# OpenDriveLab/Vista

Measured on AMD Instinct MI355X. Metric: denoise steps/sec, 25-frame 576x1024 latent, 50-step EDM @ 1/2/4/8 GPU, higher is better.
Workload: dtype bf16; 1 GPU; 1xMI355X single GPU: 25x576x1024 (latent 25x4x72x128), 50-step EulerEDM, VanillaCFG 2.5 (N=50 images per UNet call), bf16, random-init 1.65B VideoUNet, synthetic latents; frames=25, cfg_images_per_call=50, sampler=EulerEDM s_churn=0, 50-step schedule, parallelism=single GPU

## Files before the change

include/vista_hip.h:

```cpp
#ifndef VISTA_HIP_H
#define VISTA_HIP_H
#include <stdint.h>
#ifdef __cplusplus
extern "C" {
#endif

enum { VK_AMODE_DENSE = 0, VK_AMODE_CONV3X3 = 1, VK_AMODE_TEMPORAL3 = 2, VK_AMODE_CONV3D = 3 };
enum { VK_EPI_LINEAR = 0, VK_EPI_GEGLU = 1, VK_EPI_TRANS = 2 };

typedef struct VkGemmDesc {
    const void* A;
    const void* Wt;
    void* out;
    const float* bias;
    const float* rowvec;
    const void* res1;
    const void* res2;
    int32_t M, N, K;
    int32_t lda, ldc, ld_res1, ld_res2, ldv, rows_per_vec;
    float alpha, beta;
    int32_t amode, epi, out_f32;
    int32_t H, Wd, Cin, Hout, Wout, stride, ups;
    int32_t T, S;
    int32_t tile_cfg;
// ... 46 lines not shown
int vk_ff_fused_bf16(const VkGemmDesc* geglu, const VkGemmDesc* out_proj, void* stream);
int vk_ff_fused_rowstat_parts(void);

int vk_groupnorm_silu_fp8(const void* x1, const void* x2, void* y8, float* scale_out, const float* gamma, const float* beta, float* stats_ws,
                          int32_t n_img, int32_t S, int32_t C1, int32_t C2, int32_t frames_per_group, float eps, int32_t silu, void* stream);

int vk_layernorm_quant_fp8(const void* x, void* q, float* scale, const float* gamma, const float* beta, int32_t rows, int32_t C, float eps,
                           void* stream);

int vk_quantize_rows_fp8(const void* x, void* q, float* scale, int32_t M, int32_t K, int64_t ldx, int64_t ldq, void* stream);

int vk_attn_spatial_bf16(const void* q, const void* k, const void* vt, void* o, int32_t n_img, int32_t heads,
                         int32_t S, int32_t ldq, int32_t ldk, int32_t ldo, float scale, void* stream);

int vk_attn_spatial_qkv_bf16(const void* q, const void* k, const void* v, void* o, int32_t n_img, int32_t heads,
                             int32_t S, int32_t ldq, int32_t ldk, int32_t ldv, int32_t ldo, float scale, void* stream);

int vk_attn_spatial_qkv_log2_bf16(const void* q, const void* k, const void* v, void* o, int32_t n_img, int32_t heads,
                                  int32_t S, int32_t ldq, int32_t ldk, int32_t ldv, int32_t ldo, void* stream);

int vk_attn_small_bf16(const void* qkv, void* o, int32_t n_img, int32_t heads, int32_t S, int32_t D, int32_t ld, int32_t k_off,
                       int32_t v_off, int32_t ldo, float scale, void* stream);

int vk_clip_preprocess_patches(const float* img, void* out, int32_t n_img, int32_t H, int32_t W, int32_t out_hw, int32_t patch, int32_t ldo,
                               float sigma_y, float sigma_x, int32_t ks_y, int32_t ks_x, const float* mean3, const float* std3, void* stream);

int vk_attn_spatial_fp8qk(const void* q8, const void* k8, const void* q_scales, const void* k_scales, const void* v, void* o, void* o8,
                          void* o_scales, int32_t n_img, int32_t heads, int32_t S, int32_t ldq8, int32_t ldk8, int32_t ldqs, int32_t ldks,
                          int32_t ldv, int32_t ldo, int32_t ldo8, int32_t ldos, float scale, void* stream);

int vk_attn_temporal_bf16(const void* qkv, void* o, int32_t B, int32_t T, int32_t S, int32_t heads, int32_t ld,
                          int32_t k_off, int32_t v_off, int32_t ldo, float scale, void* stream);

int vk_softmax_rows_f32_bf16(const float* x, void* y, int64_t rows, int32_t cols, int64_t ldx, int64_t ldy, void* stream);

int vk_groupnorm_silu_bf16(const void* x, void* y, const float* gamma, const float* beta, float* stats_ws,
                           int32_t n_img, int32_t S, int32_t C, int32_t frames_per_group, float eps, int32_t silu,
                           void* stream);

int vk_groupnorm_stats_bf16(const void* x, float* sums, float* partial_ws, int32_t n_img, int32_t S, int32_t C,
                            int32_t frames_per_group, void* stream);
int vk_groupnorm_apply_bf16(const void* x, void* y, const float* gamma, const float* beta, const float* sums, int32_t n_img,
                            int32_t S, int32_t C, int32_t frames_per_group, float count, float eps, int32_t silu, void* stream);
int vk_groupnorm_finalize_partials(float* partial, float* sums, int32_t n_img, int32_t nchunks, int32_t frames_per_group, void* stream);
int vk_groupnorm_fold_max(void);
int vk_groupnorm_apply_partials_bf16(const void* x, void* y, const float* gamma, const float* beta, const float* partial, int32_t n_img,
                                     int32_t S, int32_t C, int32_t nchunks, int32_t frames_per_group, float count, float eps, int32_t silu,
                                     void* stream);

int vk_layernorm_bf16(const void* x, void* y, void* sum_out, const float* gamma, const float* beta,
                      const float* addvec, int32_t rows, int32_t C, int32_t rows_per_vec, int32_t ldv, float eps,
                      void* stream);

int vk_rowstats_bf16(const void* x, float* stats, int32_t rows, int32_t C, int64_t ldx, void* stream);

int vk_groupnorm_silu_cat_bf16(const void* x1, const void* x2, void* y, const float* gamma, const float* beta, float* stats_ws,
                               int32_t n_img, int32_t S, int32_t C1, int32_t C2, int32_t frames_per_group, float eps, int32_t silu,
                               void* stream);

int vk_concat_channels_bf16(const void* a, const void* b, void* out, int64_t rows, int32_t C1, int32_t C2, void* stream);

int vk_nchw_to_tokens_bf16(const float* x, void* out, int32_t n_img, int32_t C, int32_t HW, int32_t Cpad, void* stream);
int vk_tokens_to_nchw_f32(const float* x, float* out, int32_t n_img, int32_t C, int32_t HW, int32_t ldx, void* stream);

int vk_timestep_embedding_bf16(const float* t, void* out, int32_t n, int32_t dim, float max_period, void* stream);
int vk_timestep_embedding_f32(const float* t, float* out, int32_t n, int32_t dim, float max_period, void* stream);
// ... 59 lines not shown
```

vista_amd/_lib.py:

```python
import ctypes as C
import os

_HERE = os.path.dirname(os.path.abspath(__file__))
ACT_DTYPE = os.environ.get("VISTA_ACT_DTYPE", "bf16").lower()
if ACT_DTYPE not in ("bf16", "fp16"):
    raise ValueError(f"VISTA_ACT_DTYPE must be 'bf16' or 'fp16', not {ACT_DTYPE!r}")
CURRENT = ACT_DTYPE
_LIB_FILES = {"bf16": "libvista_hip.so", "fp16": "libvista_hip_f16.so"}
LIB_PATH = os.environ.get("VISTA_HIP_LIB") or os.path.join(_HERE, "lib", _LIB_FILES[ACT_DTYPE])


def lib_path(dtype_name):
    return LIB_PATH if dtype_name == ACT_DTYPE else os.path.join(_HERE, "lib", _LIB_FILES[dtype_name])


_vp = C.c_void_p
_i32 = C.c_int32
_i64 = C.c_int64
_f32 = C.c_float


class VkFp8Args(C.Structure):
    _fields_ = [("a_scale", _vp), ("w_scale", _vp), ("k_real", _i32), ("a_mx", _vp), ("ld_mx", _i32), ("mx_out", _vp), ("ld_mx_out", _i32),
                ("a_scale_rows", _i32)]
# ... 23 lines not shown

class VkRowBox(C.Structure):
    _fields_ = [("src_row", _i64), ("dst_row", _i64), ("src_stride_b", _i64), ("src_stride_t", _i64), ("dst_stride_b", _i64), ("dst_stride_t", _i64),
                ("nb", _i32), ("nt", _i32), ("ns", _i32), ("reserved", _i32)]


class VkRowBoxes(C.Structure):
    _fields_ = [("n", _i32), ("reserved", _i32), ("box", VkRowBox * VK_RESHARD_MAX_BOXES)]


ABI_VERSION = 9

SIGNATURES = {
    "vk_gemm_bf16": [C.POINTER(VkGemmDesc), _vp],
    "vk_gemm_rowstat_parts": [C.POINTER(VkGemmDesc)],
    "vk_gemm_tile_choice": [C.POINTER(VkGemmDesc)],
    "vk_gemm_tail_split": [C.POINTER(VkGemmDesc)],
    "vk_gemm_gnstat_fit": [C.POINTER(VkGemmDesc)],
    "vk_gemm_fp8": [C.POINTER(VkGemmDesc), _vp, _vp, _i32, _vp],
    "vk_gemm_fp8_mx": [C.POINTER(VkGemmDesc), C.POINTER(VkFp8Args), _vp],
    "vk_gemm_fp8_rowstat_parts": [C.POINTER(VkGemmDesc)],
    "vk_ff_fused_bf16": [C.POINTER(VkGemmDesc), C.POINTER(VkGemmDesc), _vp],
    "vk_ff_fused_rowstat_parts": [],
    "vk_layernorm_quant_fp8": [_vp, _vp, _vp, _vp, _vp, _i32, _i32, _f32, _vp],
    "vk_groupnorm_silu_fp8": [_vp, _vp, _vp, _vp, _vp, _vp, _vp, _i32, _i32, _i32, _i32, _i32, _f32, _i32, _vp],
    "vk_quantize_rows_fp8": [_vp, _vp, _vp, _i32, _i32, _i64, _i64, _vp],
    "vk_attn_spatial_bf16": [_vp, _vp, _vp, _vp, _i32, _i32, _i32, _i32, _i32, _i32, _f32, _vp],
    "vk_attn_spatial_qkv_bf16": [_vp, _vp, _vp, _vp, _i32, _i32, _i32, _i32, _i32, _i32, _i32, _f32, _vp],
    "vk_attn_spatial_qkv_log2_bf16": [_vp, _vp, _vp, _vp, _i32, _i32, _i32, _i32, _i32, _i32, _i32, _vp],
    "vk_attn_spatial_fp8qk": [_vp, _vp, _vp, _vp, _vp, _vp, _vp, _vp, _i32, _i32, _i32, _i32, _i32, _i32, _i32, _i32, _i32, _i32, _i32, _f32, _vp],
    "vk_attn_small_bf16": [_vp, _vp, _i32, _i32, _i32, _i32, _i32, _i32, _i32, _i32, _f32, _vp],
    "vk_clip_preprocess_patches": [_vp, _vp, _i32, _i32, _i32, _i32, _i32, _i32, _f32, _f32, _i32, _i32, C.POINTER(_f32), C.POINTER(_f32), _vp],
    "vk_attn_temporal_bf16": [_vp, _vp, _i32, _i32, _i32, _i32, _i32, _i32, _i32, _i32, _f32, _vp],
    "vk_softmax_rows_f32_bf16": [_vp, _vp, _i64, _i32, _i64, _i64, _vp],
    "vk_groupnorm_silu_bf16": [_vp, _vp, _vp, _vp, _vp, _i32, _i32, _i32, _i32, _f32, _i32, _vp],
    "vk_groupnorm_stats_bf16": [_vp, _vp, _vp, _i32, _i32, _i32, _i32, _vp],
    "vk_groupnorm_apply_bf16": [_vp, _vp, _vp, _vp, _vp, _i32, _i32, _i32, _i32, _f32, _f32, _i32, _vp],
    "vk_groupnorm_finalize_partials": [_vp, _vp, _i32, _i32, _i32, _vp],
    "vk_groupnorm_fold_max": [],
    "vk_groupnorm_apply_partials_bf16": [_vp, _vp, _vp, _vp, _vp, _i32, _i32, _i32, _i32, _i32, _f32, _f32, _i32, _vp],
    "vk_layernorm_bf16": [_vp, _vp, _vp, _vp, _vp, _vp, _i32, _i32, _i32, _i32, _f32, _vp],
    "vk_rowstats_bf16": [_vp, _vp, _i32, _i32, _i64, _vp],
    "vk_groupnorm_silu_cat_bf16": [_vp, _vp, _vp, _vp, _vp, _vp, _i32, _i32, _i32, _i32, _i32, _f32, _i32, _vp],
    "vk_concat_channels_bf16": [_vp, _vp, _vp, _i64, _i32, _i32, _vp],
    "vk_nchw_to_tokens_bf16": [_vp, _vp, _i32, _i32, _i32, _i32, _vp],
    "vk_tokens_to_nchw_f32": [_vp, _vp, _i32, _i32, _i32, _i32, _vp],
    "vk_timestep_embedding_bf16": [_vp, _vp, _i32, _i32, _f32, _vp],
    "vk_timestep_embedding_f32": [_vp, _vp, _i32, _i32, _f32, _vp],
    "vk_emb_combine": [_vp, _vp, _vp, _vp, _vp, _vp, _i32, _i32, _vp],
    "vk_silu_f32_to_bf16": [_vp, _vp, _i64, _vp],
    "vk_cast_f32_to_bf16": [_vp, _vp, _i64, _vp],
    "vk_sampler_prepare": [_vp, _vp, _vp, _vp, _vp, _vp, _i32, _i32, _i32, _f32, _i32, _vp],
    "vk_sampler_update": [_vp, _vp, _vp, _i32, _i32, _i32, _f32, _f32, _f32, _f32, _vp],
    "vk_denoiser_combine": [_vp, _vp, _vp, _vp, _vp, _i32, _i32, _vp],
    "vk_cfg_combine": [_vp, _vp, _vp, _i32, _i32, _vp],
    "vk_euler_step": [_vp, _vp, _vp, _vp, _vp, _i32, _i32, _vp],
    "vk_mask_replace": [_vp, _vp, _vp, _vp, _i32, _i32, _vp],
    "vk_scale_rows": [_vp, _vp, _vp, _i32, _i32, _vp],
    "vk_gaussian_sample": [_vp, _vp, _vp, _i32, _i32, _i32, _f32, _vp],
    "vk_ensemble_variance_sum": [_vp, _vp, _vp, _i32, _i64, _vp],
    "vk_lanczos_resize_u8": [_vp, _vp, _vp, _vp, _vp, _i32, _vp, _vp, _i32, _vp, _i32, _i32, _i32, _i32, _i32, _i32, _i32, _i32, _i32, _vp],
    "vk_frames_to_u8": [_vp, _vp, _i32, _i32, _i32, _i32, _i32, _i32, _vp],
    "vk_ensemble_frame_stats": [_vp, _vp, _vp, _vp, _i32, _i32, _i32, _i32, _vp],
    "vk_heat_overlay_u8": [_vp, _vp, _vp, _i32, _i32, _i32, _i32, _f32, _f32, _vp],
    "vk_copy_row_boxes": [_vp, _vp, C.POINTER(VkRowBoxes), _i64, _i64, _i32, _vp],
    "vk_abi_version": [],
# ... 39 lines not shown
```

vista_amd/build.py:

```python
import os
import subprocess
import sys

ROOT = os.path.dirname(os.path.abspath(__file__))
REPO = os.path.dirname(ROOT)
CSRC = os.path.join(ROOT, "csrc")
LIBDIR = os.path.join(ROOT, "lib")
LIB = os.path.join(LIBDIR, "libvista_hip.so")
EXTRA_FLAGS = {"ff_fused.hip": ["-fno-slp-vectorize"], "attention.hip": ["-fno-slp-vectorize"]}
SOURCES = ["gemm.hip", "gemm_pipe.hip", "gemm_pipe2.hip", "gemm_stream.hip", "gemm_fp8.hip", "ff_fused.hip", "attention.hip", "norm.hip", "elementwise.hip", "image_io.hip", "reshard.hip", "reward.hip"]


def hipcc():
    for c in (os.environ.get("HIPCC"), "/opt/rocm/bin/hipcc", "hipcc"):
        if c and (os.path.isabs(c) and os.path.exists(c) or not os.path.isabs(c)):
            return c
    raise RuntimeError("hipcc not found")


VARIANTS = {"bf16": ("libvista_hip.so", "", []), "fp16": ("libvista_hip_f16.so", "_f16", ["-DVK_F16=1"])}
LIB_F16 = os.path.join(LIBDIR, VARIANTS["fp16"][0])


def needs_build(lib=LIB):
    if not os.path.exists(lib):
        return True
    t = os.path.getmtime(lib)
    deps = [os.path.join(CSRC, f) for f in os.listdir(CSRC)] + [os.path.join(REPO, "include", "vista_hip.h")]
    return any(os.path.getmtime(d) > t for d in deps)


def build(force=False, verbose=True, variants=("bf16", "fp16")):
    os.makedirs(LIBDIR, exist_ok=True)
    procs, links = [], []
    for v in variants:
        libname, suffix, defs = VARIANTS[v]
        lib = os.path.join(LIBDIR, libname)
        if not force and not needs_build(lib):
            continue
        objs = []
        for s in SOURCES:
            o = os.path.join(LIBDIR, s.replace(".hip", suffix + ".o"))
            cmd = [hipcc(), "--offload-arch=gfx950", "-O3", "-std=c++17", "-fPIC", "-I" + os.path.join(REPO, "include"),
# ... 28 lines not shown
```

vista_amd/modules/diffusionmodules/sampling.py:

```python
import os
from typing import Dict, Union

import torch

from ... import ops
from ...util import append_dims, default, instantiate_from_config
from .guiders import IdentityGuider


class FusedDenoiser:

    def __init__(self, denoiser, network):
        self.denoiser, self.network = denoiser, network

    def __call__(self, x, sigma, cond, cond_mask):
        return self.denoiser(self.network, x, sigma, cond, cond_mask)


class BaseDiffusionSampler:
    def __init__(self, discretization_config: Union[Dict, None], num_steps: Union[int, None] = None,
                 guider_config: Union[Dict, None] = None, verbose: bool = False, device: str = "cuda"):
        self.num_steps = num_steps
        self.discretization = instantiate_from_config(discretization_config)
        self.guider = instantiate_from_config(default(guider_config, {"target": "vista_amd.modules.diffusionmodules.guiders.IdentityGuider"}))
# ... 51 lines not shown
                and self._fused_layout_ok(denoiser, x, cond, uc):
            return self._sample_fused(denoiser, x, cond, uc, cond_frame, maskf, replace, sig)
        n = x.shape[0]
        xw = x.float()
        for i in range(num_sigmas - 1):
            if replace:
                xw = ops.mask_replace(xw, cond_frame.float(), maskf)
            gamma = min(self.s_churn / (num_sigmas - 1), 2 ** 0.5 - 1) if self.s_tmin <= sig[i] <= self.s_tmax else 0.0
            s_cur = torch.full((n,), sig[i], device=x.device)
            s_next = torch.full((n,), sig[i + 1], device=x.device)
            xw = self.sampler_step(s_cur, s_next, denoiser, xw, cond, maskf, uc, gamma)
        if replace:
            xw = ops.mask_replace(xw, cond_frame.float(), maskf)
        return xw.to(x.dtype)

    @staticmethod
    def _fused_layout_ok(fd, x, cond, uc):
        if x.dim() != 4 or x.shape[1] != 4 or getattr(fd.network.diffusion_model, "in_channels", None) != 8:
            return False
        for d in (cond, uc):
            if d is None or any(k not in d for k in ("concat", "crossattn", "vector")):
                return False
            c = d["concat"]
            if c.dim() != 4 or tuple(c.shape[1:]) != tuple(x.shape[1:]):
                return False
        return True

    def _sample_fused(self, fd, x, cond, uc, cond_frame, maskf, replace, sig):
        loop = FusedLoop(self, fd, x.float().clone(), cond, uc, cond_frame, maskf, replace, sig, shard=getattr(self, "shard", None),
                         graph=self.graph, cfg_streams=self.cfg_streams)
        for i in range(len(sig) - 1):
            loop.step(i)
        return loop.finish().to(x.dtype)


class FusedLoop:

    def __init__(self, sampler, fd, xw, cond, uc, cond_frame, maskf, replace, sig, shard=None, graph=None, cfg_streams=None):
        from .video_model import CIN_PAD
        self.cin_pad = CIN_PAD
        import os
        want = os.environ.get("VISTA_HIPGRAPH", "0") if graph is None else ("1" if graph else "0")
        self._graph_mode = want
        self._graph = None
        self.den, self.unet = fd.denoiser, fd.network.diffusion_model
        self.sig, self.replace, self.shard = sig, replace, shard
        n, _, self.H, self.W = xw.shape
        self.n, self.T = n, self.den.num_frames
        T, dev = self.T, xw.device
        scales = sampler.guider.frame_scales(T).float().repeat(n // T).to(dev)
        if shard is not None and n != T:
            raise NotImplementedError("frame sharding handles one window (b = 1) per call")
        loc = (lambda t: t) if shard is None else (lambda t: shard.take_local_frames(t).contiguous())
        self.xw, self.maskf, self.scales = loc(xw), loc(maskf), loc(scales)

        def both(k):
            a, b = uc[k], cond[k]
            if a.shape[0] != n:
                a, b = a.repeat_interleave(T, 0), b.repeat_interleave(T, 0)
            return a, b
        cu, cc = both("concat")
        self.cu, self.cc = loc(cu.float().contiguous()), loc(cc.float().contiguous())
        self.half = None if shard is None else shard.cfg_half
        self.unet_shard = shard if (shard is not None and (shard.P > 1 or getattr(shard, "always_exchange", False))) else None
        if self.half is None:
            self.ctx2 = torch.cat(both("crossattn"), 0)
# ... 31 lines not shown
        n = self.n
        half = lambda t, h: t[h * n:(h + 1) * n]
        if not graph:
            ts = torch.full((n,), c_noise, device=self.xw.device)
            return torch.cat([self.unet.forward_tokens(half(net_in, h), ts, half(self.ctx2, h), half(self.y2, h), half(self.mask2, h), self.T, self.H, self.W)
                              for h in (0, 1)])
        gs = self._graph
        if gs is None:
            gs = self._graph = [self._graph_for(half(net_in, h), n, ctx=half(self.ctx2, h), y=half(self.y2, h), mask=half(self.mask2, h), slot=h) for h in (0, 1)]
        for h in (0, 1):
            gs[h]["in"].copy_(half(net_in, h))
            gs[h]["ts"].fill_(c_noise)
        dev = net_in.device
        side = FusedLoop._CFG_STREAMS.get(dev.index)
        if side is None:
            side = FusedLoop._CFG_STREAMS[dev.index] = torch.cuda.Stream(device=dev)
        cur = torch.cuda.current_stream()
        side.wait_stream(cur)
        with torch.cuda.stream(side):
            gs[1]["graph"].replay()
        gs[0]["graph"].replay()
        cur.wait_stream(side)
        return torch.cat([gs[0]["out"], gs[1]["out"]])

    _WARM_STREAMS = {}
    _CFG_STREAMS = {}

    def _graph_for(self, net_in, n_ts, ctx=None, y=None, mask=None, slot=0):
        unet = self.unet
        cache = unet.__dict__.setdefault("_hipgraph_cache", {})
        from .. import attention as _att
        if ctx is None:
            ctx, y, mask = self.ctx2, self.y2, self.mask2
        switches = (tuple(sorted(_att.FP8.items())), _att.FF_FUSED, _att.QKV_SPLIT, _att.Q_LOG2, ops.TILE_CFG, ops.GN_EPI,
                    None if self.unet_shard is None else getattr(self.unet_shard, "a2a_chunks", None))
        key = (tuple(net_in.shape), n_ts, tuple(ctx.shape), tuple(y.shape), tuple(mask.shape), self.T, self.H, self.W,
               None if self.unet_shard is None else id(self.unet_shard), str(net_in.device), switches, slot)
        g = cache.get(key)
        wkey = (_att.pack_generation(),) + tuple((id(q), _att.Packable._param_version(q)) for q in unet.parameters())
        if g is not None and g["wkey"] != wkey:
            g = None
        if g is None:
            if ops.PROFILE_ATTN is not None:
                raise RuntimeError("ops.PROFILE_ATTN records timing events around attention launches; clear it before capturing a hipGraph")
            dev = net_in.device
            g = {"in": torch.empty_like(net_in), "ts": torch.empty((n_ts,), device=dev), "ctx": ctx.clone(), "y": y.clone(),
                 "mask": mask.clone(), "wkey": wkey}
            g["in"].copy_(net_in)
            g["ts"].fill_(0.0)
            fwd = lambda: unet.forward_tokens(g["in"], g["ts"], g["ctx"], g["y"], g["mask"], self.T, self.H, self.W, shard=self.unet_shard)
            side = FusedLoop._WARM_STREAMS.get(dev.index)
            if side is None:
                side = FusedLoop._WARM_STREAMS[dev.index] = torch.cuda.Stream(device=dev)
            with ops.graph_workspace(slot):
                side.wait_stream(torch.cuda.current_stream())
                with torch.cuda.stream(side):
                    fwd()
                torch.cuda.current_stream().wait_stream(side)
                g["wkey"] = (_att.pack_generation(),) + tuple((id(q), _att.Packable._param_version(q)) for q in unet.parameters())
                g["ws"] = ops.graph_workspace_tensor()
                g["graph"] = torch.cuda.CUDAGraph()
                mode = "global" if self.unet_shard is None else "thread_local"
                with torch.cuda.graph(g["graph"], capture_error_mode=mode):
                    g["out"] = fwd()
            cache[key] = g
        else:
            g["ctx"].copy_(ctx)
            g["y"].copy_(y)
# ... 19 lines not shown
```

vista_amd/modules/video_attention.py:

```python
import torch
import torch.nn as nn

from .. import ops
from .attention import FeedForward, MemoryEfficientCrossAttention, Packable, SpatialTransformer
from .diffusionmodules.util import AlphaBlender, LayerNorm, Linear, SiLU, mlp_f32, timestep_embedding


class VideoTransformerBlock(nn.Module, Packable):
    ATTENTION_MODES = {"softmax": MemoryEfficientCrossAttention, "softmax-xformers": MemoryEfficientCrossAttention}

    def __init__(self, dim, n_heads, d_head, dropout=0.0, context_dim=None, gated_ff=True, use_checkpoint=False, timesteps=None,
                 ff_in=False, inner_dim=None, attn_mode="softmax", disable_self_attn=False, disable_temporal_crossattention=False,
                 switch_temporal_ca_to_sa=False, add_lora=False, action_control=False):
        super().__init__()
        attn_cls = self.ATTENTION_MODES[attn_mode]
        self.ff_in = ff_in or inner_dim is not None
        if inner_dim is None:
            inner_dim = dim
        assert int(n_heads * d_head) == inner_dim
        self.is_res = inner_dim == dim
        if not self.is_res:
            raise NotImplementedError("inner_dim != dim is not the Vista configuration")
        if disable_self_attn or switch_temporal_ca_to_sa:
            raise NotImplementedError("disable_self_attn / switch_temporal_ca_to_sa are not used by Vista")
        if self.ff_in:
            self.norm_in = LayerNorm(dim)
            self.ff_in = FeedForward(dim, dim_out=inner_dim, dropout=dropout, glu=gated_ff)
        self.timesteps = timesteps
        self.disable_self_attn = False
        self.attn1 = attn_cls(query_dim=inner_dim, heads=n_heads, dim_head=d_head, dropout=dropout, causal=False, add_lora=add_lora)
        self.attn1.temporal = True
        self.ff = FeedForward(inner_dim, dim_out=dim, dropout=dropout, glu=gated_ff)
        self.has_cross = not disable_temporal_crossattention
        if self.has_cross:
            self.norm2 = LayerNorm(inner_dim)
            self.attn2 = attn_cls(query_dim=inner_dim, context_dim=context_dim, heads=n_heads, dim_head=d_head, dropout=dropout,
                                  add_lora=add_lora, action_control=action_control)
        self.norm1 = LayerNorm(inner_dim)
        self.norm3 = LayerNorm(inner_dim)
        self.switch_temporal_ca_to_sa = False
        self.use_checkpoint = use_checkpoint
        self.n_heads, self.dim = n_heads, dim

    def _pack(self, dev):
        a = self.attn1
        return {"ffin_in": self.ff_in.pack_in_folded(self.norm_in, dev),
                "qkv": ops.pack_linear_cat([a.to_q.weight, a.to_k.weight, a.to_v.weight], dev, ln=self.norm1),
                "ff_in": self.ff.pack_in_folded(self.norm3, dev)}

    def forward(self, x_mix, stats, emb_rows, clip_context, B, T, S, alpha, emit_stats=False):
        assert self.timesteps is None or self.timesteps == T
        if not self.ff_in:
            raise NotImplementedError("extra_ff_mix_layer=False is not the Vista configuration")
        pk = self.packed()
        a1 = self.attn1.packed()
        x, st = self.ff_in.forward_folded(x_mix, stats, pk["ffin_in"], self.norm_in, res1=x_mix, emit_stats=True)
        qkv = ops.linear(x, pk["qkv"], ln=st, alt_cols_from=2 * x.shape[-1])
        att = ops.attn_temporal(qkv, B, T, S, self.n_heads, self.attn1.dim_head ** -0.5)
        if self.has_cross:
            cv = self.attn2.context_vector(clip_context)
            x, st = ops.linear(att, a1["out"], res1=x, rowvec=cv, rows_per_vec=T * S, emit_stats=True)
        else:
            x, st = ops.linear(att, a1["out"], res1=x, emit_stats=True)
        r = self.ff.forward_folded(x, st, pk["ff_in"], self.norm3, res1=x, alpha=1.0 - alpha, res2=x_mix, rowvec2=emb_rows.neg_rows,
                                   beta=alpha, rows_per_vec=S, emit_stats=emit_stats)
        return r if emit_stats else (r, None)


class _EmbRows:

    __slots__ = ("rows", "neg_rows")

    def __init__(self, rows):
        self.rows, self.neg_rows = rows, rows.neg()


class SpatialVideoTransformer(SpatialTransformer):

    def __init__(self, in_channels, n_heads, d_head, depth=1, dropout=0.0, use_linear=False, context_dim=None,
                 use_spatial_context=False, timesteps=None, merge_strategy="fixed", merge_factor=0.5, time_context_dim=None,
                 ff_in=False, use_checkpoint=False, time_depth=1, attn_mode="softmax", disable_self_attn=False,
                 disable_temporal_crossattention=False, max_time_embed_period=10000, add_lora=False, action_control=False):
        super().__init__(in_channels, n_heads, d_head, depth=depth, dropout=dropout, attn_type=attn_mode, use_checkpoint=use_checkpoint,
                         context_dim=context_dim, use_linear=use_linear, disable_self_attn=disable_self_attn, add_lora=add_lora,
                         action_control=action_control)
        self.time_depth = time_depth
        self.depth = depth
        self.max_time_embed_period = max_time_embed_period
        inner_dim = n_heads * d_head
        if not use_spatial_context:
            raise NotImplementedError("use_spatial_context=False (separate time_context) is not the Vista configuration")
# ... 65 lines not shown
```

vista_amd/ops.py:

```python
import ctypes as C
import math
import os
import threading

import torch

from . import _lib
from ._lib import VkFp8Args, VkGemmDesc, check

AMODE_DENSE, AMODE_CONV3X3, AMODE_TEMPORAL3, AMODE_CONV3D = 0, 1, 2, 3
EPI_LINEAR, EPI_GEGLU, EPI_TRANS = 0, 1, 2
ACT = torch.float16 if _lib.ACT_DTYPE == "fp16" else torch.bfloat16
BF16 = ACT
F32 = torch.float32


class storage:

    def __init__(self, dtype):
        if dtype not in (torch.bfloat16, torch.float16):
            raise ValueError("ops.storage: torch.bfloat16 or torch.float16")
        self.dtype, self.name = dtype, ("fp16" if dtype is torch.float16 else "bf16")

    def __enter__(self):
# ... 87 lines not shown
    return (norm.weight, norm.bias, norm.eps)


KPERM16 = (0, 1, 2, 3, 8, 9, 10, 11, 4, 5, 6, 7, 12, 13, 14, 15)


def pack_linear(weight, bias=None, device="cuda", ln=None):
    return _finish_pack(weight.detach().reshape(weight.shape[0], -1).float(), None if bias is None else bias.detach().float(), device,
                        ln=None if ln is None else _ln_tuple(ln))


def ff_out_layout(w):
    N, K = w.shape
    if K % 32:
        raise ValueError("ff_out_layout needs K % 32 == 0")
    w = w.reshape(N, K // 16, 16)[:, :, list(KPERM16)].reshape(N, K // 32, 32)
    return w.permute(1, 0, 2).contiguous().reshape(K // 32 * N, 32)


def pack_ff_out(weight, bias=None, device="cuda"):
    w = weight.detach().reshape(weight.shape[0], -1).float()
    N, K = w.shape
    b = None if bias is None else bias.detach().to(device=device, dtype=F32).contiguous()
    return PackedWeight(ff_out_layout(w).to(device=device, dtype=BF16), b, N, K, ffout=True)


def pack_rows_as_weight(t, N, K):
    _need(t, BF16, "t")
    return PackedWeight(t, None, N, K)


def pack_linear_cat(weights, device="cuda", ln=None):
    return _finish_pack(torch.cat([w.detach().float() for w in weights], 0), None, device, ln=None if ln is None else _ln_tuple(ln))


def geglu_perm(nout):
    if nout % 16:
        raise ValueError("GEGLU width must be a multiple of 16")
    idx = torch.arange(nout).reshape(-1, 16)
    return torch.stack([idx, idx + nout], 1).reshape(-1)


def pack_geglu(weight, bias, device="cuda", ln=None):
    w = weight.detach().float()
    b = bias.detach().float()
    perm = geglu_perm(w.shape[0] // 2).to(w.device)
    return _finish_pack(w[perm], b[perm], device, geglu=True, ln=None if ln is None else _ln_tuple(ln))


def _slab_major(w):
    cout, taps, cin = w.shape
    return w.reshape(cout, taps, cin // 64, 64).permute(0, 2, 1, 3).reshape(cout, taps * cin)


def pack_conv3x3(weight, bias=None, cin_pad=None, device="cuda"):
    w = weight.detach().float().permute(0, 2, 3, 1).contiguous()
    cout, _, _, cin = w.shape
    cp = cin_pad or ceil_to(cin, 64)
    if cp != cin:
        w = torch.nn.functional.pad(w, (0, cp - cin))
    return _finish_pack(_slab_major(w.reshape(cout, 9, cp)), None if bias is None else bias.detach().float(), device)


def pack_conv_t3(weight, bias=None, device="cuda", cin_pad=None):
    w = weight.detach().float()[:, :, :, 0, 0].permute(0, 2, 1).contiguous()
    cout, _, cin = w.shape
# ... 629 lines not shown


CLIP_MEAN = (0.48145466, 0.4578275, 0.40821073)
CLIP_STD = (0.26862954, 0.26130258, 0.27577711)


def clip_preprocess_patches(img, out_hw=224, patch=14, kpad=None, antialias=True, mean=CLIP_MEAN, std=CLIP_STD):
    _need(img, F32, "img")
    img = img.contiguous()
    n, c, H, W = img.shape
    if c != 3:
        raise ValueError("clip_preprocess_patches: 3-channel images")
    g = out_hw // patch
    kp = kpad or ceil_to(3 * patch * patch, 64)
    out = torch.zeros((n * (1 + g * g), kp), dtype=BF16, device=img.device)
    down = antialias and max(H / out_hw, W / out_hw) > 1
    (sy, ky), (sx, kx) = (antialias_blur_params(H, out_hw), antialias_blur_params(W, out_hw)) if down else ((1.0, 1), (1.0, 1))
    m3, s3 = (C.c_float * 3)(*mean), (C.c_float * 3)(*std)
    check(_lib.load().vk_clip_preprocess_patches(_p(img), _p(out), n, H, W, out_hw, patch, kp, sy, sx, ky, kx, m3, s3, _stream()),
          "vk_clip_preprocess_patches")
    return out


def attn_temporal(qkv, B, T, S, heads, scale=None):
    _need(qkv, BF16, "qkv")
    c = heads * 64
    o = torch.empty((B * T * S, c), dtype=BF16, device=qkv.device)
    lib = _lib.load()
    check(lib.vk_attn_temporal_bf16(_p(qkv), _p(o), B, T, S, heads, qkv.stride(0), c, 2 * c, o.stride(0),
                                    float(scale if scale is not None else 1.0 / math.sqrt(64)), _stream()), "vk_attn_temporal_bf16")
    return o


def softmax_rows(x, out=None):
    _need(x, F32, "x")
    rows, cols = x.shape
    if x.stride(1) != 1:
        raise ValueError("softmax_rows: rows must be contiguous")
    if out is None:
        out = torch.empty((rows, cols), dtype=BF16, device=x.device)
    check(_lib.load().vk_softmax_rows_f32_bf16(_p(x), _p(out), rows, cols, x.stride(0), out.stride(0), _stream()), "vk_softmax_rows_f32_bf16")
    return out


def _gn_partials_ok(gn, n_img, S, Cc):
    if gn is None or gn.t is None:
        return False
    if gn.rows != n_img * S or gn.C != Cc or gn.nchunks * 64 != S:
        raise ValueError(f"GnPartials of a ({gn.rows} rows, {gn.C} channels, {gn.nchunks * 64} rows per image) tensor passed to a GroupNorm over ({n_img}, {S}, {Cc})")
    return True


def groupnorm(x, gamma, beta, eps, silu, frames_per_group=1, out=None, gn=None):
    _need(x, BF16, "x")
    if not x.is_contiguous():
        raise ValueError("groupnorm: x must be contiguous")
    n_img, S, Cc = x.shape
    if out is None:
        out = torch.empty_like(x)
    if _gn_partials_ok(gn, n_img, S, Cc):
        lib = _lib.load()
        count = float(Cc // 32) * float(S) * float(frames_per_group)
        if frames_per_group * gn.nchunks <= lib.vk_groupnorm_fold_max():
            check(lib.vk_groupnorm_apply_partials_bf16(_p(x), _p(out), _p(gamma), _p(beta), _p(gn.t), n_img, S, Cc, gn.nchunks, frames_per_group, count,
                                                       float(eps), 1 if silu else 0, _stream()), "vk_groupnorm_apply_partials_bf16")
            gn.t = None
# ... 331 lines not shown
```

Before: 6.341 steps/s.

## Fuse temporal attention QKV projection with attention in one kernel

Adds a HIP kernel that computes the LayerNorm-folded QKV projection for one head and a group of pixels into LDS, then runs the per-pixel temporal softmax attention straight from that staged tile. Weights are repacked head-interleaved (q,k,v per head) so each block's 192-column slice holds one head's q, k and v. This removes the global write and re-read of the full QKV tensor and one kernel launch per temporal block when K ≤ 640 and T ≤ 32. The cost is a second packed weight copy, less tiling freedom than the generic GEMM, and a GEMM tile of 256 rows that wastes rows when 256 is not a multiple of T (25 frames gives 10 pixels, 250 rows).

```diff
diff --git a/include/vista_hip.h b/include/vista_hip.h
--- a/include/vista_hip.h
+++ b/include/vista_hip.h
@@ -102,6 +102,10 @@
 int vk_attn_temporal_bf16(const void* qkv, void* o, int32_t B, int32_t T, int32_t S, int32_t heads, int32_t ld,
                           int32_t k_off, int32_t v_off, int32_t ldo, float scale, void* stream);
 
+int vk_attn_temporal_qkv_bf16(const VkGemmDesc* proj, void* o, int32_t B, int32_t T, int32_t S, int32_t heads, int32_t ldo, float scale,
+                              void* stream);
+int vk_attn_temporal_qkv_fit(const VkGemmDesc* proj, int32_t B, int32_t T, int32_t S, int32_t heads);
+
 int vk_softmax_rows_f32_bf16(const float* x, void* y, int64_t rows, int32_t cols, int64_t ldx, int64_t ldy, void* stream);
 
 int vk_groupnorm_silu_bf16(const void* x, void* y, const float* gamma, const float* beta, float* stats_ws,
diff --git a/vista_amd/_lib.py b/vista_amd/_lib.py
--- a/vista_amd/_lib.py
+++ b/vista_amd/_lib.py
@@ -79,6 +79,8 @@
     "vk_attn_small_bf16": [_vp, _vp, _i32, _i32, _i32, _i32, _i32, _i32, _i32, _i32, _f32, _vp],
     "vk_clip_preprocess_patches": [_vp, _vp, _i32, _i32, _i32, _i32, _i32, _i32, _f32, _f32, _i32, _i32, C.POINTER(_f32), C.POINTER(_f32), _vp],
     "vk_attn_temporal_bf16": [_vp, _vp, _i32, _i32, _i32, _i32, _i32, _i32, _i32, _i32, _f32, _vp],
+    "vk_attn_temporal_qkv_bf16": [C.POINTER(VkGemmDesc), _vp, _i32, _i32, _i32, _i32, _i32, _f32, _vp],
+    "vk_attn_temporal_qkv_fit": [C.POINTER(VkGemmDesc), _i32, _i32, _i32, _i32],
     "vk_softmax_rows_f32_bf16": [_vp, _vp, _i64, _i32, _i64, _i64, _vp],
     "vk_groupnorm_silu_bf16": [_vp, _vp, _vp, _vp, _vp, _i32, _i32, _i32, _i32, _f32, _i32, _vp],
     "vk_groupnorm_stats_bf16": [_vp, _vp, _vp, _i32, _i32, _i32, _i32, _vp],
diff --git a/vista_amd/build.py b/vista_amd/build.py
--- a/vista_amd/build.py
+++ b/vista_amd/build.py
@@ -8,7 +8,7 @@
 LIBDIR = os.path.join(ROOT, "lib")
 LIB = os.path.join(LIBDIR, "libvista_hip.so")
 EXTRA_FLAGS = {"ff_fused.hip": ["-fno-slp-vectorize"], "attention.hip": ["-fno-slp-vectorize"]}
-SOURCES = ["gemm.hip", "gemm_pipe.hip", "gemm_pipe2.hip", "gemm_stream.hip", "gemm_fp8.hip", "ff_fused.hip", "attention.hip", "norm.hip", "elementwise.hip", "image_io.hip", "reshard.hip", "reward.hip"]
+SOURCES = ["gemm.hip", "gemm_pipe.hip", "gemm_pipe2.hip", "gemm_stream.hip", "gemm_fp8.hip", "ff_fused.hip", "attention.hip", "attn_temporal_qkv.hip", "norm.hip", "elementwise.hip", "image_io.hip", "reshard.hip", "reward.hip"]
 
 
 def hipcc():
diff --git a/vista_amd/csrc/attn_temporal_qkv.hip b/vista_amd/csrc/attn_temporal_qkv.hip
--- /dev/null
+++ b/vista_amd/csrc/attn_temporal_qkv.hip
@@ -0,0 +1,291 @@
+#include "common.h"
+#include "vista_hip.h"
+
+#include "gemm_common.h"
+
+namespace {
+
+constexpr int QBM = 256, QBN = 192, QNT = 512;
+constexpr int QFX = 3, QFY = 2;
+constexpr int QA_BYTES = QBM * 128, QSTAGE = (QBM + QBN) * 128;
+constexpr int Q_LN_OFF = 2 * QSTAGE, Q_EV_OFF = Q_LN_OFF + QBM * 8, Q_SMEM = Q_EV_OFF + 2 * QBN * 4;
+constexpr int QROW = 400;
+static_assert(QBM * QROW <= 2 * QSTAGE, "the staged tile overlays the stage buffers");
+
+constexpr float TQ_LOG2E = 1.4426950408889634f;
+constexpr float TQ_NEG_BIG = -1.0e30f;
+
+__device__ uint4 g_tq_zero16;
+
+__device__ __forceinline__ float tq_exp2(float x) { return __builtin_amdgcn_exp2f(x); }
+
+template <bool WIDE>
+__device__ __forceinline__ void tq_attend(const char* __restrict__ rows , uint16_t* __restrict__ o,
+                                          const size_t row0, const int T, const int S, const int ldo, const int head, const float scale_log2,
+                                          const int l31, const int lh) {
+    const bool t_ok = l31 < T;
+    bf16x8_t qf[4], kf[4];
+    {
+        const char* rp = rows + (t_ok ? l31 : 0) * QROW + 16 * lh;
+#pragma unroll
+        for (int ks = 0; ks < 4; ++ks) {
+            uint4 a = *(const uint4*)(rp + 32 * ks);
+            uint4 c = *(const uint4*)(rp + 128 + 32 * ks);
+            if (!t_ok) { a = make_uint4(0, 0, 0, 0); c = make_uint4(0, 0, 0, 0); }
+            qf[ks] = __builtin_bit_cast(bf16x8_t, a);
+            kf[ks] = __builtin_bit_cast(bf16x8_t, c);
+        }
+    }
+    f32x16_t sacc;
+#pragma unroll
+    for (int r = 0; r < 16; ++r) sacc[r] = 0.f;
+#pragma unroll
+    for (int ks = 0; ks < 4; ++ks) sacc = vk_mfma(kf[ks], qf[ks], sacc);
+
+    float mx = TQ_NEG_BIG;
+#pragma unroll
+    for (int r = 0; r < 16; ++r) {
+        const int key = (r & 3) + 8 * (r >> 2) + 4 * lh;
+        if (key >= T) sacc[r] = TQ_NEG_BIG;
+        mx = fmaxf(mx, sacc[r]);
+    }
+    mx = fmaxf(mx, __shfl_xor(mx, 32, 64));
+    const float mb = mx * scale_log2;
+    float psum = 0.f;
+#pragma unroll
+    for (int r = 0; r < 16; ++r) {
+        const int key = (r & 3) + 8 * (r >> 2) + 4 * lh;
+        float pv = tq_exp2(fmaf(sacc[r], scale_log2, -mb));
+        if (key >= T) pv = 0.f;
+        sacc[r] = pv;
+        psum += pv;
+    }
+    psum += __shfl_xor(psum, 32, 64);
+    const float inv = 1.f / psum;
+
+    bf16x8_t pf[2];
+#pragma unroll
+    for (int J = 0; J < 2; ++J) {
+        uint4 v;
+        v.x = pack_bf16x(sacc[8 * J + 0], sacc[8 * J + 1]);
+        v.y = pack_bf16x(sacc[8 * J + 2], sacc[8 * J + 3]);
+        v.z = pack_bf16x(sacc[8 * J + 4], sacc[8 * J + 5]);
+        v.w = pack_bf16x(sacc[8 * J + 6], sacc[8 * J + 7]);
+        pf[J] = __builtin_bit_cast(bf16x8_t, v);
+    }
+
+    f32x16_t oacc[2];
+#pragma unroll
+    for (int d = 0; d < 2; ++d) {
+#pragma unroll
+        for (int r = 0; r < 16; ++r) oacc[d][r] = 0.f;
+#pragma unroll
+        for (int J = 0; J < 2; ++J) {
+            uint32_t w[4];
+#pragma unroll
+            for (int i2 = 0; i2 < 4; ++i2) {
+                const int ka = 16 * J + 8 * ((2 * i2) >> 2) + 4 * lh + ((2 * i2) & 3);
+                const char* vp = rows + 256 + (32 * d + l31) * 2;
+                const uint16_t lo = ka < T ? *(const uint16_t*)(vp + ka * QROW) : (uint16_t)0;
+                const uint16_t hi = ka + 1 < T ? *(const uint16_t*)(vp + (ka + 1) * QROW) : (uint16_t)0;
+                w[i2] = (uint32_t)lo | ((uint32_t)hi << 16);
+            }
+            const uint4 v = make_uint4(w[0], w[1], w[2], w[3]);
+            oacc[d] = vk_mfma_bf16x(__builtin_bit_cast(bf16x8_t, v), pf[J], oacc[d]);
+        }
+    }
+    if (WIDE) {
+        uint16_t* optr = o + (row0 + (size_t)(t_ok ? l31 : 0) * S) * ldo + head * 64 + 8 * lh;
+#pragma unroll
+        for (int d = 0; d < 2; ++d)
+#pragma unroll
+            for (int gp = 0; gp < 2; ++gp) {
+                uint2 qa, qb;
+                qa.x = pack_bf16(oacc[d][8 * gp + 0] * inv, oacc[d][8 * gp + 1] * inv);
+                qa.y = pack_bf16(oacc[d][8 * gp + 2] * inv, oacc[d][8 * gp + 3] * inv);
+                qb.x = pack_bf16(oacc[d][8 * gp + 4] * inv, oacc[d][8 * gp + 5] * inv);
+                qb.y = pack_bf16(oacc[d][8 * gp + 6] * inv, oacc[d][8 * gp + 7] * inv);
+                const auto rx = __builtin_amdgcn_permlane32_swap(qa.x, qb.x, false, false);
+                const auto ry = __builtin_amdgcn_permlane32_swap(qa.y, qb.y, false, false);
+                if (t_ok) *(uint4*)(optr + 32 * d + 16 * gp) = make_uint4(rx[0], ry[0], rx[1], ry[1]);
+            }
+    } else if (t_ok) {
+        uint16_t* optr = o + (row0 + (size_t)l31 * S) * ldo + head * 64 + 4 * lh;
+#pragma unroll
+        for (int d = 0; d < 2; ++d)
+#pragma unroll
+            for (int g = 0; g < 4; ++g) {
+                uint2 w2;
+                w2.x = pack_bf16(oacc[d][4 * g + 0] * inv, oacc[d][4 * g + 1] * inv);
+                w2.y = pack_bf16(oacc[d][4 * g + 2] * inv, oacc[d][4 * g + 3] * inv);
+                *(uint2*)(optr + 32 * d + 8 * g) = w2;
+            }
+    }
+}
+
+template <bool WIDE>
+__global__ __launch_bounds__(QNT, 2) void attn_temporal_qkv_kernel(const VkGemmDesc p, uint16_t* __restrict__ o, const int B, const int T, const int S,
+                                                                    const int heads, const int ldo, const float scale_log2, const int P,
+                                                                    const int ngroups) {
+    __shared__ __attribute__((aligned(16))) char smem[Q_SMEM];
+    typedef const __attribute__((address_space(1))) void* gptr_t;
+    typedef __attribute__((address_space(3))) void* lptr_t;
+
+    const int tid = threadIdx.x;
+    const int lane = tid & 63, wave = tid >> 6;
+    const int wm = wave >> 1, wn = wave & 1;
+    const int l31 = lane & 31, lh = lane >> 5;
+    const int wave_u = __builtin_amdgcn_readfirstlane(wave);
+
+    const int logical = xcd_remap(blockIdx.x, ngroups * heads);
+    const int grp = logical / heads, head = logical - grp * heads;
+    const long long npix = (long long)B * S;
+    const long long g0 = (long long)grp * P;
+
+    auto src_row = [&](const int r) -> long long {
+        const int pp = r / T, t = r - pp * T;
+        const long long g = g0 + pp;
+        if (pp >= P || g >= npix) return -1;
+        const long long b = g / S, s = g - b * S;
+        return (b * T + t) * S + s;
+    };
+
+    const int lc = tid & 7, lr = tid >> 3;
+    const int lsrc = lc ^ ((lr >> 1) & 7);
+    const char* asrc[4];
+#pragma unroll
+    for (int i = 0; i < 4; ++i) {
+        const long long m = src_row(lr + 64 * i);
+        asrc[i] = m < 0 ? nullptr : (const char*)((const uint16_t*)p.A + (size_t)m * p.lda + lsrc * 8);
+    }
+    const char* const wsrc = (const char*)((const uint16_t*)p.Wt + ((size_t)head * QBN + lr) * p.K + lsrc * 8);
+    const size_t wpass = (size_t)64 * p.K * 2;
+    auto dma = [&](const int kt, const int stage) __attribute__((always_inline)) {
+        char* const sA = smem + stage * QSTAGE + wave_u * 1024;
+#pragma unroll
+        for (int i = 0; i < 4; ++i) {
+            const char* s = asrc[i] ? asrc[i] + kt * (BK * 2) : (const char*)&g_tq_zero16;
+            __builtin_amdgcn_global_load_lds((gptr_t)s, (lptr_t)(sA + i * 64 * 128), 16, 0, 0);
+        }
+#pragma unroll
+        for (int i = 0; i < 3; ++i)
+            __builtin_amdgcn_global_load_lds((gptr_t)(wsrc + i * wpass + kt * (BK * 2)), (lptr_t)(sA + QA_BYTES + i * 64 * 128), 16, 0, 0);
+    };
+
+    float2* const lnrow = (float2*)(smem + Q_LN_OFF);
+    float* const ev = (float*)(smem + Q_EV_OFF);
+
+    dma(0, 0);
+    if (tid < QBM) {
+        const long long m = src_row(tid);
+        lnrow[tid] = ln_row_stats(p, (int)(m < 0 ? 0 : m));
+    }
+    if (tid < 2 * QBN) {
+        const int c = tid < QBN ? tid : tid - QBN;
+        const float* src = tid < QBN ? p.bias : p.ln_colsum;
+        ev[tid] = src ? src[head * QBN + c] : 0.f;
+    }
+    __syncthreads();
+
+    f32x16_t acc[QFX][QFY];
+#pragma unroll
+    for (int i = 0; i < QFX; ++i)
+#pragma unroll
+        for (int j = 0; j < QFY; ++j)
+#pragma unroll
+            for (int r = 0; r < 16; ++r) acc[i][j][r] = 0.f;
+
+    const int sw = (l31 >> 1) & 7;
+    const int xrow = QA_BYTES + (wn * (QFX * 32) + l31) * 128, yrow = (wm * (QFY * 32) + l31) * 128;
+    const int nk = p.K / BK;
+    int st = 0;
+    for (int kt = 0; kt < nk; ++kt) {
+        if (kt + 1 < nk) dma(kt + 1, st ^ 1);
+#pragma unroll
+        for (int ks = 0; ks < 4; ++ks) {
+            const char* sb = smem + st * QSTAGE + (((ks * 2 + lh) ^ sw) << 4);
+            bf16x8_t xf[QFX], yf[QFY];
+#pragma unroll
+            for (int f = 0; f < QFY; ++f) yf[f] = *(const bf16x8_t*)(sb + yrow + f * 32 * 128);
+#pragma unroll
+            for (int f = 0; f < QFX; ++f) xf[f] = *(const bf16x8_t*)(sb + xrow + f * 32 * 128);
+#pragma unroll
+            for (int fi = 0; fi < QFX; ++fi)
+#pragma unroll
+                for (int fj = 0; fj < QFY; ++fj) acc[fi][fj] = vk_mfma(xf[fi], yf[fj], acc[fi][fj]);
+        }
+        __syncthreads();
+        st ^= 1;
+    }
+
+#pragma unroll
+    for (int fj = 0; fj < QFY; ++fj) {
+        const int row = wm * (QFY * 32) + fj * 32 + l31;
+        const float2 t = lnrow[row];
+        const float rs = t.y, nrm = -t.x * t.y;
+        char* const trow = smem + row * QROW;
+#pragma unroll
+        for (int fi = 0; fi < QFX; ++fi) {
+            const bool vcols = wn * QFX + fi >= 4;
+            uint2 packed[4];
+#pragma unroll
+            for (int g = 0; g < 4; ++g) {
+                const int c = wn * (QFX * 32) + fi * 32 + 8 * g + 4 * lh;
+                const float4 b = *(const float4*)(ev + c);
+                const float4 cs = *(const float4*)(ev + QBN + c);
+                float v[4];
+#pragma unroll
+                for (int e = 0; e < 4; ++e) v[e] = acc[fi][fj][4 * g + e];
+                v[0] = fmaf(rs, v[0], fmaf(nrm, cs.x, b.x)); v[1] = fmaf(rs, v[1], fmaf(nrm, cs.y, b.y));
+                v[2] = fmaf(rs, v[2], fmaf(nrm, cs.z, b.z)); v[3] = fmaf(rs, v[3], fmaf(nrm, cs.w, b.w));
+                packed[g].x = vcols ? pack_bf16x(v[0], v[1]) : pack_bf16(v[0], v[1]);
+                packed[g].y = vcols ? pack_bf16x(v[2], v[3]) : pack_bf16(v[2], v[3]);
+            }
+#pragma unroll
+            for (int gp = 0; gp < 2; ++gp) {
+                const uint4 w = widen_pair(packed[2 * gp], packed[2 * gp + 1]);
+                *(uint4*)(trow + (wn * (QFX * 32) + fi * 32 + 16 * gp + 8 * lh) * 2) = w;
+            }
+        }
+    }
+    __syncthreads();
+
+    for (int pp = wave_u; pp < P; pp += QNT / 64) {
+        const long long g = g0 + pp;
+        if (g >= npix) break;
+        const long long b = g / S, s = g - b * S;
+        tq_attend<WIDE>(smem + pp * T * QROW, o, (size_t)(b * T * S + s), T, S, ldo, head, scale_log2, l31, lh);
+    }
+}
+
+}
+
+extern "C" int vk_attn_temporal_qkv_fit(const VkGemmDesc* d, int32_t B, int32_t T, int32_t S, int32_t heads) {
+    if (!d || B <= 0 || S <= 0 || heads <= 0 || T < 1 || T > 32) return 0;
+    if (d->amode != AMODE_DENSE || d->epi != EPI_LINEAR || d->A2 || !d->A || !d->Wt) return 0;
+    if (d->K <= 0 || (d->K % BK) != 0 || d->lda < d->K || (d->lda % 8) != 0 || (((size_t)d->A) & 15) != 0 || (((size_t)d->Wt) & 15) != 0) return 0;
+    if ((long long)d->N != (long long)heads * QBN || (long long)d->M != (long long)B * T * S) return 0;
+    if (!d->ln_stats || !d->ln_colsum || d->ln_parts <= 0 || d->ln_parts > 64 || !(d->ln_eps > 0.f)) return 0;
+    if (d->res1 || d->res2 || d->rowvec || d->rowvec2 || d->act || d->rowstat_out || d->out_f32 || d->mx8_out || d->gnstat_out) return 0;
+    if (d->alpha != 1.f) return 0;
+    if (d->m_begin != 0 || (d->m_end != 0 && d->m_end != d->M)) return 0;
+    const long long ngroups = ((long long)B * S + (QBM / T) - 1) / (QBM / T);
+    if (ngroups * heads > 0x7fffffffLL) return 0;
+    return 1;
+}
+
+extern "C" int vk_attn_temporal_qkv_bf16(const VkGemmDesc* proj, void* o, int32_t B, int32_t T, int32_t S, int32_t heads, int32_t ldo, float scale,
+                                         void* stream_) {
+    if (!proj || !o || !vk_attn_temporal_qkv_fit(proj, B, T, S, heads)) return VK_EINVAL;
+    if ((ldo % 4) != 0 || ldo < heads * 64 || (((size_t)o) & 7) != 0) return VK_EINVAL;
+    const int P = QBM / T;
+    const int ngroups = (int)(((long long)B * S + P - 1) / P);
+    const bool wide = (ldo % 8) == 0 && (((size_t)o) & 15) == 0;
+#define VK_TQ(WD) hipLaunchKernelGGL((attn_temporal_qkv_kernel<WD>), dim3(ngroups * heads), dim3(QNT), 0, (hipStream_t)stream_, *proj, (uint16_t*)o, B, T, \
+                                     S, heads, ldo, scale * TQ_LOG2E, P, ngroups)
+    if (wide) VK_TQ(true);
+    else VK_TQ(false);
+#undef VK_TQ
+    VK_CHECK_LAUNCH();
+    return VK_OK;
+}
diff --git a/vista_amd/modules/diffusionmodules/sampling.py b/vista_amd/modules/diffusionmodules/sampling.py
--- a/vista_amd/modules/diffusionmodules/sampling.py
+++ b/vista_amd/modules/diffusionmodules/sampling.py
@@ -107,6 +107,13 @@
         for i in range(len(sig) - 1):
             loop.step(i)
         return loop.finish().to(x.dtype)
+
+
+def launch_switches(unet_shard=None):
+    from .. import attention as _att
+    from .. import video_attention as _vatt
+    return (tuple(sorted(_att.FP8.items())), _att.FF_FUSED, _att.QKV_SPLIT, _att.Q_LOG2, ops.TILE_CFG, ops.GN_EPI, _vatt.TATTN_QKV,
+            None if unet_shard is None else getattr(unet_shard, "a2a_chunks", None))
 
 
 class FusedLoop:
@@ -204,8 +211,7 @@
         from .. import attention as _att
         if ctx is None:
             ctx, y, mask = self.ctx2, self.y2, self.mask2
-        switches = (tuple(sorted(_att.FP8.items())), _att.FF_FUSED, _att.QKV_SPLIT, _att.Q_LOG2, ops.TILE_CFG, ops.GN_EPI,
-                    None if self.unet_shard is None else getattr(self.unet_shard, "a2a_chunks", None))
+        switches = launch_switches(self.unet_shard)
         key = (tuple(net_in.shape), n_ts, tuple(ctx.shape), tuple(y.shape), tuple(mask.shape), self.T, self.H, self.W,
                None if self.unet_shard is None else id(self.unet_shard), str(net_in.device), switches, slot)
         g = cache.get(key)
diff --git a/vista_amd/modules/video_attention.py b/vista_amd/modules/video_attention.py
--- a/vista_amd/modules/video_attention.py
+++ b/vista_amd/modules/video_attention.py
@@ -1,9 +1,14 @@
+import os
+
 import torch
 import torch.nn as nn
 
 from .. import ops
 from .attention import FeedForward, MemoryEfficientCrossAttention, Packable, SpatialTransformer
 from .diffusionmodules.util import AlphaBlender, LayerNorm, Linear, SiLU, mlp_f32, timestep_embedding
+
+
+TATTN_QKV = os.environ.get("VISTA_TATTN_QKV", "1") != "0"
 
 
 class VideoTransformerBlock(nn.Module, Packable):
@@ -43,10 +48,18 @@
         self.n_heads, self.dim = n_heads, dim
 
     def _pack(self, dev):
-        a = self.attn1
         return {"ffin_in": self.ff_in.pack_in_folded(self.norm_in, dev),
-                "qkv": ops.pack_linear_cat([a.to_q.weight, a.to_k.weight, a.to_v.weight], dev, ln=self.norm1),
                 "ff_in": self.ff.pack_in_folded(self.norm3, dev)}
+
+    def _qkv_pack(self, pk, fused, dev):
+        name = "qkv_heads" if fused else "qkv"
+        pw = pk.get(name)
+        if pw is None:
+            a = self.attn1
+            ws = [a.to_q.weight, a.to_k.weight, a.to_v.weight]
+            with torch.no_grad():
+                pw = pk[name] = ops.pack_qkv_heads(ws, self.n_heads, dev, ln=self.norm1) if fused else ops.pack_linear_cat(ws, dev, ln=self.norm1)
+        return pw
 
     def forward(self, x_mix, stats, emb_rows, clip_context, B, T, S, alpha, emit_stats=False):
         assert self.timesteps is None or self.timesteps == T
@@ -55,8 +68,16 @@
         pk = self.packed()
         a1 = self.attn1.packed()
         x, st = self.ff_in.forward_folded(x_mix, stats, pk["ffin_in"], self.norm_in, res1=x_mix, emit_stats=True)
-        qkv = ops.linear(x, pk["qkv"], ln=st, alt_cols_from=2 * x.shape[-1])
-        att = ops.attn_temporal(qkv, B, T, S, self.n_heads, self.attn1.dim_head ** -0.5)
+        scale = self.attn1.dim_head ** -0.5
+        fused = False
+        if TATTN_QKV and self.attn1.dim_head == 64 and x.shape[-1] <= ops.TATTN_QKV_MAX_K:
+            pwh = self._qkv_pack(pk, True, x.device)
+            fused = ops.attn_temporal_qkv_fit(x, pwh, st, B, T, S, self.n_heads)
+        if fused:
+            att = ops.attn_temporal_qkv(x, pwh, st, B, T, S, self.n_heads, scale)
+        else:
+            qkv = ops.linear(x, self._qkv_pack(pk, False, x.device), ln=st, alt_cols_from=2 * x.shape[-1])
+            att = ops.attn_temporal(qkv, B, T, S, self.n_heads, scale)
         if self.has_cross:
             cv = self.attn2.context_vector(clip_context)
             x, st = ops.linear(att, a1["out"], res1=x, rowvec=cv, rows_per_vec=T * S, emit_stats=True)
diff --git a/vista_amd/ops.py b/vista_amd/ops.py
--- a/vista_amd/ops.py
+++ b/vista_amd/ops.py
@@ -143,6 +143,27 @@
 
 def pack_linear_cat(weights, device="cuda", ln=None):
     return _finish_pack(torch.cat([w.detach().float() for w in weights], 0), None, device, ln=None if ln is None else _ln_tuple(ln))
+
+
+def qkv_head_perm(heads, d_head=64):
+    c = heads * d_head
+    idx = torch.arange(c).reshape(heads, d_head)
+    return torch.stack([idx, idx + c, idx + 2 * c], 1).reshape(-1)
+
+
+def pack_qkv_heads(weights, heads, device="cuda", ln=None):
+    pw = pack_linear_cat(weights, device, ln=ln)
+    perm = qkv_head_perm(heads)
+    n = perm.numel()
+    if pw.N != n:
+        raise ValueError(f"pack_qkv_heads: {pw.N} rows for {heads} heads of 64")
+    perm = perm.to(pw.wt.device)
+    pw.wt[:n] = pw.wt[:n][perm]
+    if pw.colsum is not None:
+        pw.colsum[:n] = pw.colsum[:n][perm]
+    if pw.bias is not None:
+        pw.bias[:n] = pw.bias[:n][perm]
+    return pw
 
 
 def geglu_perm(nout):
@@ -838,6 +859,42 @@
     return o
 
 
+TATTN_QKV_MAX_K = 640
+
+
+def _tattn_qkv_desc(x, pw, ln, B, T, S, heads):
+    _need(x, BF16, "x")
+    x2d, lda = _rows2d(x, "x")
+    M = x2d.shape[0]
+    if x2d.shape[1] != pw.K:
+        raise ValueError(f"attn_temporal_qkv: K mismatch {x2d.shape[1]} vs {pw.K}")
+    d = VkGemmDesc()
+    d.A, d.lda = _p(x2d), lda
+    d.amode, d.epi = AMODE_DENSE, EPI_LINEAR
+    d.Wt, d.bias = _p(pw.wt), _p(pw.bias)
+    d.M, d.N, d.K = M, pw.N, pw.K
+    d.alpha = 1.0
+    _fill_ln(d, pw, ln, M)
+    return d
+
+
+def attn_temporal_qkv_fit(x, pw, ln, B, T, S, heads):
+    if pw.K > TATTN_QKV_MAX_K:
+        return False
+    d = _tattn_qkv_desc(x, pw, ln, B, T, S, heads)
+    return _lib.load().vk_attn_temporal_qkv_fit(C.byref(d), B, T, S, heads) == 1
+
+
+def attn_temporal_qkv(x, pw, ln, B, T, S, heads, scale=None, out=None):
+    d = _tattn_qkv_desc(x, pw, ln, B, T, S, heads)
+    o = out if out is not None else torch.empty((B * T * S, heads * 64), dtype=BF16, device=x.device)
+    if out is not None:
+        _need(out, BF16, "out")
+    check(_lib.load().vk_attn_temporal_qkv_bf16(C.byref(d), _p(o), B, T, S, heads, o.stride(0),
+                                                float(scale if scale is not None else 1.0 / math.sqrt(64)), _stream()), "vk_attn_temporal_qkv_bf16")
+    return o
+
+
 def softmax_rows(x, out=None):
     _need(x, F32, "x")
     rows, cols = x.shape
```

New measurement: 6.401 steps/s (median of 6 runs). About the same (+0.9%).
